# phazei/ComfyUI-HunyuanVideo-Foley

Hardware: AMD Instinct MI355X
Metric: audio-sec/sec (5s clip, 50-step Euler, CFG 4.5) (higher is better)
Workload: dtype bf16; 1 GPU; c2: T2A 5 s, 50 Euler steps, CFG 4.5, hunyuanvideo-foley-xxl, bs=1/GPU, bf16 GEMM operands / fp32 accumulate, weight storage none, DAC-VAE fp32 decode to 48 kHz, host-to-host (H2D noise + D2H waveform timed); clips_per_gpu=1, parallelism=dp1, hip_graph=True, progress_callback=False, collectives=0, bundle_bytes=10565004032, rccl_nranks=1

## Files before the change

comfyui-hunyuanvideo-foley_amd/csrc/attention.hip:

```cpp
#include <type_traits>

#include "kernels.h"

namespace {


template <int HD> __device__ constexpr float attn_scale() {
  return HD == 128 ? 0.08838834764831845f : HD == 64 ? 0.125f : 0.10206207261596575f;
}

__device__ __forceinline__ void attn_block_coords(const AttnArgs& a, int qtile, int& qt, int& h, int& b) {
  const int nq = (a.Sq + qtile - 1) / qtile;
  const int nwg = nq * a.H * a.Bq;
  int bid = (int)blockIdx.x;
  const int xcd = bid & 7, slot = bid >> 3;
  const int q = nwg >> 3, r = nwg & 7;
  bid = ((xcd < r) ? xcd * (q + 1) : r * (q + 1) + (xcd - r) * q) + slot;
  qt = bid % nq;
  const int bh = bid / nq;
  h = bh % a.H;
  b = bh / a.H;
}

template <typename OutT> struct Pack4Out;
template <> struct Pack4Out<float> {
  static __device__ __forceinline__ void store(float* p, const f32x4 v) { *(f32x4*)p = v; }
};
template <> struct Pack4Out<bf16_t> {
  static __device__ __forceinline__ void store(bf16_t* p, const f32x4 v) {
    uint2 w;
    w.x = pack_bf16x2(v[0], v[1]);
    w.y = pack_bf16x2(v[2], v[3]);
    *(uint2*)p = w;
  }
};

template <> struct Pack4Out<f16_t> {
  static __device__ __forceinline__ void store(f16_t* p, const f32x4 v) {
    uint2 w;
    w.x = pack_f16x2(v[0], v[1]);
    w.y = pack_f16x2(v[2], v[3]);
    *(uint2*)p = w;
  }
};

template <typename OutT, int HD>
__global__ __launch_bounds__(64) void attn_kernel(const AttnArgs a) {
  const int lane = threadIdx.x;
  const int j = lane & 31, kh = lane >> 5;
  const int q0 = blockIdx.x * 32;
  const int h = blockIdx.y, b = blockIdx.z;
  const int bk = b / a.kv_bdiv;
  const float* __restrict__ Q = (const float*)a.q + ((long)(b * a.H + h) * a.Sq) * HD;
  const float* __restrict__ K = (const float*)a.k + ((long)(bk * a.H + h) * a.Skv) * HD;
  const float* __restrict__ V = (const float*)a.v + ((long)(bk * a.H + h) * a.Skv) * HD;
  const float scale = attn_scale<HD>();

  constexpr int HH = HD / 2, NC = HD / 8;
  float qr[HH];
  {
    const int qrow = min(q0 + j, a.Sq - 1);
    const f32x4* p = (const f32x4*)(Q + (long)qrow * HD + kh * HH);
#pragma unroll
    for (int c = 0; c < NC; ++c) {
      const f32x4 v = p[c];
      qr[c * 4 + 0] = v[0]; qr[c * 4 + 1] = v[1]; qr[c * 4 + 2] = v[2]; qr[c * 4 + 3] = v[3];
    }
  }

  constexpr int ND = HD / 32;
  f32x16 o[ND];
#pragma unroll
  for (int d = 0; d < ND; ++d)
#pragma unroll
    for (int e = 0; e < 16; ++e) o[d][e] = 0.f;
  float m_run = -INFINITY, l_run = 0.f;

  for (int kt = 0; kt < a.Skv; kt += 32) {
    f32x16 s;
#pragma unroll
    for (int e = 0; e < 16; ++e) s[e] = 0.f;
    {
      const int krow = min(kt + j, a.Skv - 1);
      const f32x4* p = (const f32x4*)(K + (long)krow * HD + kh * HH);
#pragma unroll
      for (int c = 0; c < NC; ++c) {
        const f32x4 v = p[c];
        s = __builtin_amdgcn_mfma_f32_32x32x2f32(v[0], qr[c * 4 + 0], s, 0, 0, 0);
        s = __builtin_amdgcn_mfma_f32_32x32x2f32(v[1], qr[c * 4 + 1], s, 0, 0, 0);
        s = __builtin_amdgcn_mfma_f32_32x32x2f32(v[2], qr[c * 4 + 2], s, 0, 0, 0);
        s = __builtin_amdgcn_mfma_f32_32x32x2f32(v[3], qr[c * 4 + 3], s, 0, 0, 0);
      }
    }
    float mx = -INFINITY;
#pragma unroll
    for (int e = 0; e < 16; ++e) {
      const int key = kt + (e & 3) + 8 * (e >> 2) + 4 * kh;
      s[e] = (key < a.Skv) ? s[e] * scale : -INFINITY;
      mx = fmaxf(mx, s[e]);
    }
    mx = xhalf_max(mx);
    const float m_new = fmaxf(m_run, mx);
    const float alpha = expf(m_run - m_new);
    float ps = 0.f;
#pragma unroll
    for (int e = 0; e < 16; ++e) {
      s[e] = expf(s[e] - m_new);
      ps += s[e];
    }
    ps = xhalf_sum(ps);
    l_run = l_run * alpha + ps;
    m_run = m_new;
#pragma unroll
    for (int d = 0; d < ND; ++d)
#pragma unroll
      for (int e = 0; e < 16; ++e) o[d][e] *= alpha;
#pragma unroll
    for (int t = 0; t < 16; ++t) {
      const int vrow = min(kt + (t & 3) + 8 * (t >> 2) + 4 * kh, a.Skv - 1);
      const float* vp = V + (long)vrow * HD + j;
#pragma unroll
      for (int d = 0; d < ND; ++d)
        o[d] = __builtin_amdgcn_mfma_f32_32x32x2f32(vp[d * 32], s[t], o[d], 0, 0, 0);
    }
  }

  const int tok = q0 + j;
  if (tok >= a.Sq) return;
  const float inv = 1.0f / l_run;
  OutT* dst;
  if (HD == 64 && a.out_rows) {
    const int orow = a.out_rows[(long)b * a.Sq + tok];
    if ((unsigned)orow >= (unsigned)a.out_nrows) return;
    dst = (OutT*)a.outA + (long)orow * (a.H * HD);
  }
  else if (tok < a.split) dst = (OutT*)a.outA + ((long)b * a.split + tok) * (a.H * HD);
  else dst = (OutT*)a.outB + ((long)b * (a.Sq - a.split) + (tok - a.split)) * (a.H * HD);
  dst += h * HD;
#pragma unroll
  for (int d = 0; d < ND; ++d)
#pragma unroll
    for (int g4 = 0; g4 < 4; ++g4) {
      const int c = d * 32 + 8 * g4 + 4 * kh;
#pragma unroll
      for (int u = 0; u < 4; ++u) dst[c + u] = Cvt<OutT>::to(o[d][g4 * 4 + u] * inv);
    }
}

template <typename T, typename OutT>
__global__ __launch_bounds__(256) void attn_bf16_kernel(const AttnArgs a) {
  constexpr int HD = 128;
  __shared__ float sO[4][3][16][64];
  __shared__ float sM[4][32], sL[4][32];
  const int lane = threadIdx.x & 63, w = threadIdx.x >> 6;
  const int j = lane & 31, kh = lane >> 5;
  int qt, h, b;
  attn_block_coords(a, 32, qt, h, b);
  const int q0 = qt * 32;
  const int bk = b / a.kv_bdiv;
  const T* __restrict__ Q = (const T*)a.q + ((long)(b * a.H + h) * a.Sq) * HD;
  const T* __restrict__ K = (const T*)a.k + ((long)(bk * a.H + h) * a.Skv) * HD;
  const T* __restrict__ VT = (const T*)a.v + ((long)(bk * a.H + h) * HD) * a.vt_pitch;
  const float scale2 = 0.08838834764831845f * 1.4426950408889634f;

  const bool stamp = a.dbg && threadIdx.x == 0;
  if (stamp) a.dbg[(long)blockIdx.x * 8 + 0] = wall_clock64();
  bf16x8 qf[8];
  {
    const T* p = Q + (long)min(q0 + j, a.Sq - 1) * HD + 8 * kh;
#pragma unroll
    for (int s = 0; s < 8; ++s) qf[s] = *(const bf16x8*)(p + 16 * s);
  }
  f32x16 o[4];
#pragma unroll
  for (int d = 0; d < 4; ++d)
#pragma unroll
    for (int e = 0; e < 16; ++e) o[d][e] = 0.f;
  float m_run = -INFINITY, l_run = 0.f;

  const int nt = (a.Skv + 31) >> 5;
  const int t0 = (nt * w) >> 2, t1 = (nt * (w + 1)) >> 2;
  const int pi = 16 * ((j >> 2) & 1) + (j & 3) + 4 * (j >> 3);
  auto tile = [&](int kt, const bf16x8 (&kf)[8], const bf16x8 (&vf)[2][4]) {
    f32x16 s;
#pragma unroll
    for (int e = 0; e < 16; ++e) s[e] = 0.f;
#pragma unroll
    for (int st = 0; st < 8; ++st) s = mfma16<T>(kf[st], qf[st], s);
    float mx = -INFINITY;
#pragma unroll
    for (int e = 0; e < 16; ++e) {
      s[e] = (kt + 16 * kh + e < a.Skv) ? s[e] * scale2 : -INFINITY;
      mx = fmaxf(mx, s[e]);
    }
    mx = xhalf_max(mx);
    const float m_new = fmaxf(m_run, mx);
    float ps = 0.f;
    bf16x8 pb[2];
#pragma unroll
    for (int e = 0; e < 16; ++e) {
      const float pv = __builtin_amdgcn_exp2f(s[e] - m_new);
      ps += pv;
      pb[e >> 3][e & 7] = to_carrier<T>(pv);
    }
    ps = xhalf_sum(ps);
    if (__builtin_amdgcn_ballot_w64(m_new > m_run) != 0) {
      const float alpha = __builtin_amdgcn_exp2f(m_run - m_new);
      l_run *= alpha;
#pragma unroll
      for (int d = 0; d < 4; ++d)
#pragma unroll
        for (int e = 0; e < 16; ++e) o[d][e] *= alpha;
    }
    l_run += ps;
    m_run = m_new;
#pragma unroll
    for (int u = 0; u < 2; ++u)
#pragma unroll
      for (int d = 0; d < 4; ++d) o[d] = mfma16<T>(vf[u][d], pb[u], o[d]);
  };
  auto load_k = [&](int kt, bf16x8 (&kf)[8]) {
    const T* p = K + (long)min(kt + pi, a.Skv - 1) * HD + 8 * kh;
#pragma unroll
    for (int st = 0; st < 8; ++st) kf[st] = *(const bf16x8*)(p + 16 * st);
  };
  auto load_v = [&](int kt, bf16x8 (&vf)[2][4]) {
#pragma unroll
    for (int u = 0; u < 2; ++u)
#pragma unroll
      for (int d = 0; d < 4; ++d) vf[u][d] = *(const bf16x8*)(VT + (long)(d * 32 + j) * a.vt_pitch + kt + 16 * kh + 8 * u);
  };
  if (t1 - t0 <= 2) {
    bf16x8 k0[8], k1[8], v0[2][4], v1[2][4];
    const int kta = t0 * 32, ktb = min(t0 + 1, nt - 1) * 32;
    if (t1 > t0) {
      load_k(kta, k0);
      load_k(ktb, k1);
      load_v(kta, v0);
      load_v(ktb, v1);
      if (a.dbg) {
        asm volatile("s_waitcnt vmcnt(0)" ::: "memory");
        if (stamp) a.dbg[(long)blockIdx.x * 8 + 1] = wall_clock64();
      }
      tile(kta, k0, v0);
      if (t1 - t0 == 2) tile(ktb, k1, v1);
    }
  } else {
    for (int t = t0; t < t1; ++t) {
      bf16x8 kf[8], vf[2][4];
      load_k(t * 32, kf);
      load_v(t * 32, vf);
      tile(t * 32, kf, vf);
    }
  }

  if (stamp) a.dbg[(long)blockIdx.x * 8 + 2] = wall_clock64();
  if (kh == 0) {
    sM[w][j] = m_run;
    sL[w][j] = l_run;
  }
#pragma unroll
  for (int d = 0; d < 4; ++d) {
    if (d == w) continue;
    const int slot = d < w ? d : d - 1;
#pragma unroll
    for (int e = 0; e < 16; ++e) sO[w][slot][e][lane] = o[d][e];
  }
  __syncthreads();
  if (stamp) a.dbg[(long)blockIdx.x * 8 + 3] = wall_clock64();
  float mstar = -INFINITY;
#pragma unroll
  for (int x = 0; x < 4; ++x) mstar = fmaxf(mstar, sM[x][j]);
  float wt[4], L = 0.f;
#pragma unroll
  for (int x = 0; x < 4; ++x) {
    wt[x] = __builtin_amdgcn_exp2f(sM[x][j] - mstar);
    L += wt[x] * sL[x][j];
  }
  const int tok = q0 + j;
  if (tok >= a.Sq) return;
  const float inv = 1.0f / L;
  OutT* dst;
  if (tok < a.split) dst = (OutT*)a.outA + ((long)b * a.split + tok) * (a.H * HD);
  else dst = (OutT*)a.outB + ((long)b * (a.Sq - a.split) + (tok - a.split)) * (a.H * HD);
  dst += h * HD + w * 32;
  const int slot_mine = 0;
  (void)slot_mine;
  auto finish = [&](auto wc) {
    constexpr int W = decltype(wc)::value;
    float part[3][16];
#pragma unroll
    for (int x = 0, n = 0; x < 4; ++x) {
      if (x == W) continue;
      const int slot = W < x ? W : W - 1;
#pragma unroll
      for (int e = 0; e < 16; ++e) part[n][e] = sO[x][slot][e][lane];
      ++n;
    }
#pragma unroll
    for (int g4 = 0; g4 < 4; ++g4) {
      f32x4 r;
#pragma unroll
      for (int u = 0; u < 4; ++u) {
        const int e = g4 * 4 + u;
        float acc = 0.f;
#pragma unroll
        for (int x = 0, n = 0; x < 4; ++x) {
          if (x == W) acc += wt[x] * o[W][e];
          else acc += wt[x] * part[n++][e];
        }
        r[u] = acc * inv;
      }
      Pack4Out<OutT>::store(dst + 8 * g4 + 4 * kh, r);
    }
  };
  switch (__builtin_amdgcn_readfirstlane(w)) {
    case 0: finish(std::integral_constant<int, 0>{}); break;
    case 1: finish(std::integral_constant<int, 1>{}); break;
    case 2: finish(std::integral_constant<int, 2>{}); break;
    default: finish(std::integral_constant<int, 3>{}); break;
  }
  if (stamp) a.dbg[(long)blockIdx.x * 8 + 4] = wall_clock64();
}

__device__ __forceinline__ void attn_buf_lds16(const void* base, unsigned bytes, unsigned char* lds_wave_base, int voff) {
  const __amdgpu_buffer_rsrc_t r = __builtin_amdgcn_make_buffer_rsrc((void*)base, 0, (int)bytes, 0x00020000);
  __builtin_amdgcn_raw_ptr_buffer_load_lds(r, (__attribute__((address_space(3))) void*)lds_wave_base, 16, voff, 0, 0, 0);
}

template <typename T, typename OutT>
__global__ __launch_bounds__(256) void attn_lds_kernel(const AttnArgs a, const int merge_off) {
  constexpr int HD = 128;
  extern __shared__ __attribute__((aligned(16))) unsigned char dsm[];
  float (*sO)[3][16][64] = (float (*)[3][16][64])(dsm + merge_off);
  float (*sM)[32] = (float (*)[32])(dsm + merge_off + 4 * 3 * 16 * 64 * 4);
  float (*sL)[32] = (float (*)[32])(dsm + merge_off + 4 * 3 * 16 * 64 * 4 + 4 * 32 * 4);
  const int lane = threadIdx.x & 63, w = threadIdx.x >> 6;
  const int j = lane & 31, kh = lane >> 5;
  int qt, h, b;
  attn_block_coords(a, 32, qt, h, b);
  const int q0 = qt * 32;
  const int bk = b / a.kv_bdiv;
  const T* __restrict__ Q = (const T*)a.q + ((long)(b * a.H + h) * a.Sq) * HD;
  const T* __restrict__ K = (const T*)a.k + ((long)(bk * a.H + h) * a.Skv) * HD;
  const T* __restrict__ VT = (const T*)a.v + ((long)(bk * a.H + h) * HD) * a.vt_pitch;
  const float scale2 = 0.08838834764831845f * 1.4426950408889634f;

  const bool stamp = a.dbg && threadIdx.x == 0;
  if (stamp) a.dbg[(long)blockIdx.x * 8 + 0] = wall_clock64();
  const int nt = (a.Skv + 31) >> 5;
  const int lgCV = a.vt_pitch > 128 ? 5 : 4;
  unsigned char* const Ks = dsm;
  unsigned char* const Vs = Ks + nt * 32 * 256;
  unsigned char* const Qs = Vs + (128 << (lgCV + 4));
  const int wv = __builtin_amdgcn_readfirstlane(w);
  {
    const int r4 = lane >> 4, c16 = lane & 15;
    for (int p = wv; p < nt * 8; p += 4) {
      const int row = 4 * p + r4;
      const int g = c16 ^ ((row & 7) | ((row >> 1) & 8));
      attn_buf_lds16(K, (unsigned)a.Skv * 256u, Ks + p * 1024, row * 256 + g * 16);
    }
    const int vchunks = a.vt_pitch >> 3;
    for (int p = wv; p < (128 << lgCV) >> 6; p += 4) {
      const int pos = p * 64 + lane;
      const int row = pos >> lgCV, g = (pos & ((1 << lgCV) - 1)) ^ (row & 15);
      attn_buf_lds16(VT, (unsigned)(HD * a.vt_pitch * 2), Vs + p * 1024, g < vchunks ? (row * a.vt_pitch + g * 8) * 2 : 0x7ffffff0);
    }
    for (int p = wv; p < 8; p += 4) {
      const int row = 4 * p + r4;
      attn_buf_lds16(Q + (long)q0 * HD, (unsigned)(a.Sq - q0) * 256u, Qs + p * 1024, row * 256 + ((c16 ^ (row & 15)) << 4));
    }
  }
  asm volatile("s_waitcnt vmcnt(0)" ::: "memory");
  __syncthreads();
  if (stamp) a.dbg[(long)blockIdx.x * 8 + 1] = wall_clock64();
  bf16x8 qf[8];
#pragma unroll
  for (int s = 0; s < 8; ++s) qf[s] = *(const bf16x8*)(Qs + j * 256 + (((2 * s + kh) ^ (j & 15)) << 4));
  f32x16 o[4];
#pragma unroll
  for (int d = 0; d < 4; ++d)
#pragma unroll
    for (int e = 0; e < 16; ++e) o[d][e] = 0.f;
  float m_run = -INFINITY, l_run = 0.f;

  const int t0 = (nt * w) >> 2, t1 = (nt * (w + 1)) >> 2;
  const int pi = 16 * ((j >> 2) & 1) + (j & 3) + 4 * (j >> 3);
  auto tile = [&](int kt, const bf16x8 (&kf)[8], const bf16x8 (&vf)[2][4]) {
    f32x16 s;
#pragma unroll
    for (int e = 0; e < 16; ++e) s[e] = 0.f;
#pragma unroll
    for (int st = 0; st < 8; ++st) s = mfma16<T>(kf[st], qf[st], s);
    float mx = -INFINITY;
#pragma unroll
    for (int e = 0; e < 16; ++e) {
      s[e] = (kt + 16 * kh + e < a.Skv) ? s[e] * scale2 : -INFINITY;
      mx = fmaxf(mx, s[e]);
    }
    mx = xhalf_max(mx);
    const float m_new = fmaxf(m_run, mx);
    float ps = 0.f;
    bf16x8 pb[2];
#pragma unroll
    for (int e = 0; e < 16; ++e) {
      const float pv = __builtin_amdgcn_exp2f(s[e] - m_new);
      ps += pv;
      pb[e >> 3][e & 7] = to_carrier<T>(pv);
    }
    ps = xhalf_sum(ps);
    if (__builtin_amdgcn_ballot_w64(m_new > m_run) != 0) {
      const float alpha = __builtin_amdgcn_exp2f(m_run - m_new);
      l_run *= alpha;
#pragma unroll
      for (int d = 0; d < 4; ++d)
#pragma unroll
        for (int e = 0; e < 16; ++e) o[d][e] *= alpha;
    }
    l_run += ps;
    m_run = m_new;
#pragma unroll
    for (int u = 0; u < 2; ++u)
#pragma unroll
      for (int d = 0; d < 4; ++d) o[d] = mfma16<T>(vf[u][d], pb[u], o[d]);
  };
  const int pk = (pi & 7) | ((pi >> 1) & 8);
  auto read_k = [&](int kt, bf16x8 (&kf)[8]) {
    const unsigned char* kr = Ks + (kt + pi) * 256;
#pragma unroll
    for (int st = 0; st < 8; ++st) kf[st] = *(const bf16x8*)(kr + (((2 * st + kh) ^ pk) << 4));
  };
  auto read_v = [&](int kt, bf16x8 (&vf)[2][4]) {
#pragma unroll
    for (int u = 0; u < 2; ++u)
#pragma unroll
      for (int d = 0; d < 4; ++d) {
        const int row = d * 32 + j;
        vf[u][d] = *(const bf16x8*)(Vs + (row << (lgCV + 4)) + ((((kt >> 3) + 2 * kh + u) ^ (row & 15)) << 4));
      }
  };
  if (t1 - t0 <= 2) {
    bf16x8 k0[8], k1[8], v0[2][4], v1[2][4];
    const int kta = t0 * 32, ktb = min(t0 + 1, nt - 1) * 32;
    if (t1 > t0) {
      read_k(kta, k0);
      read_k(ktb, k1);
      read_v(kta, v0);
      read_v(ktb, v1);
      tile(kta, k0, v0);
      if (t1 - t0 == 2) tile(ktb, k1, v1);
    }
  } else {
    for (int t = t0; t < t1; ++t) {
      bf16x8 kf[8], vf[2][4];
      read_k(t * 32, kf);
      read_v(t * 32, vf);
      tile(t * 32, kf, vf);
    }
  }

  if (stamp) a.dbg[(long)blockIdx.x * 8 + 2] = wall_clock64();
  if (merge_off == 0) __syncthreads();
  if (kh == 0) {
    sM[w][j] = m_run;
    sL[w][j] = l_run;
  }
#pragma unroll
  for (int d = 0; d < 4; ++d) {
    if (d == w) continue;
    const int slot = d < w ? d : d - 1;
#pragma unroll
    for (int e = 0; e < 16; ++e) sO[w][slot][e][lane] = o[d][e];
  }
  __syncthreads();
  if (stamp) a.dbg[(long)blockIdx.x * 8 + 3] = wall_clock64();
  float mstar = -INFINITY;
#pragma unroll
  for (int x = 0; x < 4; ++x) mstar = fmaxf(mstar, sM[x][j]);
  float wt[4], L = 0.f;
#pragma unroll
  for (int x = 0; x < 4; ++x) {
    wt[x] = __builtin_amdgcn_exp2f(sM[x][j] - mstar);
    L += wt[x] * sL[x][j];
  }
  const int tok = q0 + j;
  if (tok >= a.Sq) return;
  const float inv = 1.0f / L;
  OutT* dst;
  if (tok < a.split) dst = (OutT*)a.outA + ((long)b * a.split + tok) * (a.H * HD);
  else dst = (OutT*)a.outB + ((long)b * (a.Sq - a.split) + (tok - a.split)) * (a.H * HD);
  dst += h * HD + w * 32;
  const int slot_mine = 0;
  (void)slot_mine;
  auto finish = [&](auto wc) {
    constexpr int W = decltype(wc)::value;
    float part[3][16];
#pragma unroll
    for (int x = 0, n = 0; x < 4; ++x) {
      if (x == W) continue;
      const int slot = W < x ? W : W - 1;
#pragma unroll
      for (int e = 0; e < 16; ++e) part[n][e] = sO[x][slot][e][lane];
      ++n;
    }
#pragma unroll
    for (int g4 = 0; g4 < 4; ++g4) {
      f32x4 r;
#pragma unroll
      for (int u = 0; u < 4; ++u) {
        const int e = g4 * 4 + u;
        float acc = 0.f;
#pragma unroll
        for (int x = 0, n = 0; x < 4; ++x) {
          if (x == W) acc += wt[x] * o[W][e];
          else acc += wt[x] * part[n++][e];
        }
        r[u] = acc * inv;
      }
      Pack4Out<OutT>::store(dst + 8 * g4 + 4 * kh, r);
    }
  };
  switch (__builtin_amdgcn_readfirstlane(w)) {
    case 0: finish(std::integral_constant<int, 0>{}); break;
    case 1: finish(std::integral_constant<int, 1>{}); break;
    case 2: finish(std::integral_constant<int, 2>{}); break;
    default: finish(std::integral_constant<int, 3>{}); break;
  }
  if (stamp) a.dbg[(long)blockIdx.x * 8 + 4] = wall_clock64();
}

template <typename T, typename OutT, int HD, bool GRP = false>
__global__ __launch_bounds__(256) __attribute__((amdgpu_waves_per_eu(3, 3))) void attn_bf16_wide_kernel(const AttnArgs a) {
  constexpr int KP = 2 * HD + 16, VP = 80;
  constexpr int STG = 32 * KP + HD * VP;
  constexpr int NS = HD / 16, ND = HD / 32;
  constexpr int CK = HD / 8, NP = HD / 64;
  __shared__ __attribute__((aligned(16))) unsigned char lds[2 * STG];
  const int tid = threadIdx.x, lane = tid & 63, w = tid >> 6;
  const int j = lane & 31, kh = lane >> 5;
  int qt, h, b;
  attn_block_coords(a, 128, qt, h, b);
  const int q0 = qt * 128 + w * 32;
  const int bk = b / a.kv_bdiv;
  const T* __restrict__ Q = (const T*)a.q + ((long)(b * a.H + h) * a.Sq) * HD;
  const T* __restrict__ K = (const T*)a.k + ((long)(bk * a.H + h) * a.Skv) * HD;
  const T* __restrict__ VT = (const T*)a.v + ((long)(bk * a.H + h) * HD) * a.vt_pitch;
  const float scale2 = attn_scale<HD>() * 1.4426950408889634f;

  bf16x8 qf[NS];
  {
    const T* p = Q + (long)min(q0 + j, a.Sq - 1) * HD + 8 * kh;
#pragma unroll
    for (int s = 0; s < NS; ++s) qf[s] = *(const bf16x8*)(p + 16 * s);
  }
  f32x16 o[ND];
#pragma unroll
  for (int d = 0; d < ND; ++d)
#pragma unroll
    for (int e = 0; e < 16; ++e) o[d][e] = 0.f;
  float m_run = -INFINITY, l_run = 0.f;
  int klo = 0, khi = 0, wlo = 0, whi = 0;
  if constexpr (GRP) {
    const int qi = min(q0 + j, a.Sq - 1);
    klo = (qi / a.grp_q) * a.grp_kv;
    khi = klo + a.grp_kv;
    if (q0 < a.Sq) {
      wlo = (q0 / a.grp_q) * a.grp_kv;
      whi = (min(q0 + 31, a.Sq - 1) / a.grp_q + 1) * a.grp_kv;
    }
  }

  const int k_row0 = tid / CK, k_col = tid % CK;
  const int v_row0 = tid >> 2, v_col = tid & 3;
  constexpr int NPX = HD % 64 ? 2 : NP;
  u32x4 rk[NPX], rv[NPX];
  auto gload = [&](int t) {
    const int kt = t * 32;
    if constexpr (HD % 64 == 0) {
#pragma unroll
      for (int i = 0; i < NP; ++i) {
        rk[i] = *(const u32x4*)(K + (long)min(kt + k_row0 + i * (256 / CK), a.Skv - 1) * HD + k_col * 8);
        rv[i] = *(const u32x4*)(VT + (long)(v_row0 + i * 64) * a.vt_pitch + kt + v_col * 8);
      }
    } else {
#pragma unroll
      for (int i = 0; i < NPX; ++i) {
        const int p = tid + 256 * i;
        if (p < 4 * HD) {
          rk[i] = *(const u32x4*)(K + (long)min(kt + p / CK, a.Skv - 1) * HD + (p % CK) * 8);
          rv[i] = *(const u32x4*)(VT + (long)(p >> 2) * a.vt_pitch + kt + (p & 3) * 8);
        }
      }
    }
  };
  auto lstore = [&](int stage) {
    unsigned char* base = lds + stage * STG;
    if constexpr (HD % 64 == 0) {
#pragma unroll
      for (int i = 0; i < NP; ++i) {
        *(u32x4*)(base + (k_row0 + i * (256 / CK)) * KP + k_col * 16) = rk[i];
        *(u32x4*)(base + 32 * KP + (v_row0 + i * 64) * VP + v_col * 16) = rv[i];
      }
    } else {
#pragma unroll
      for (int i = 0; i < NPX; ++i) {
        const int p = tid + 256 * i;
        if (p < 4 * HD) {
          *(u32x4*)(base + (p / CK) * KP + (p % CK) * 16) = rk[i];
          *(u32x4*)(base + 32 * KP + (p >> 2) * VP + (p & 3) * 16) = rv[i];
        }
      }
    }
  };
  const int nt = (a.Skv + 31) >> 5;
  const int pi = 16 * ((j >> 2) & 1) + (j & 3) + 4 * (j >> 3);
  const bool acct = a.dbg && tid == 0;
  long long c_math = 0, c_stage = 0, c_t0 = acct ? (long long)__builtin_readcyclecounter() : 0;
  gload(0);
  lstore(0);
  __syncthreads();
  for (int t = 0; t < nt; ++t) {
    const int kt = t * 32;
    const long long ca = acct ? (long long)__builtin_readcyclecounter() : 0;
    if (t + 1 < nt) gload(t + 1);
    const unsigned char* Ks = lds + (t & 1) * STG;
    const unsigned char* Vs = Ks + 32 * KP;
    bool live = true;
    if constexpr (GRP) live = kt < whi && kt + 32 > wlo;
    if (live) {
    f32x16 s;
#pragma unroll
    for (int e = 0; e < 16; ++e) s[e] = 0.f;
#pragma unroll
    for (int st = 0; st < NS; ++st)
      s = mfma16<T>(*(const bf16x8*)(Ks + pi * KP + (16 * st + 8 * kh) * 2), qf[st], s);
    float mx = -INFINITY;
    if constexpr (GRP) {
#pragma unroll
      for (int e = 0; e < 16; ++e) {
        const int key = kt + 16 * kh + e;
        s[e] = (key >= klo && key < khi) ? s[e] : -INFINITY;
      }
    } else if (kt + 32 > a.Skv) {
#pragma unroll
      for (int e = 0; e < 16; ++e) s[e] = (kt + 16 * kh + e < a.Skv) ? s[e] : -INFINITY;
    }
#pragma unroll
    for (int e = 0; e < 16; ++e) mx = fmaxf(mx, s[e]);
    mx = xhalf_max(mx);
    const float m_new = fmaxf(m_run, mx * scale2);
    const float m_exp = (GRP && m_new == -INFINITY) ? 0.f : m_new;
    float ps = 0.f;
    bf16x8 pb[2];
#pragma unroll
    for (int e = 0; e < 16; ++e) {
      const float pv = __builtin_amdgcn_exp2f(__builtin_fmaf(s[e], scale2, -m_exp));
      ps += pv;
      pb[e >> 3][e & 7] = to_carrier<T>(pv);
    }
    ps = xhalf_sum(ps);
    if (__builtin_amdgcn_ballot_w64(m_new > m_run) != 0) {
      const float alpha = (GRP && m_new == -INFINITY) ? 1.f : __builtin_amdgcn_exp2f(m_run - m_new);
      l_run *= alpha;
#pragma unroll
      for (int d = 0; d < ND; ++d)
#pragma unroll
        for (int e = 0; e < 16; ++e) o[d][e] *= alpha;
    }
    l_run += ps;
    m_run = m_new;
#pragma unroll
    for (int u = 0; u < 2; ++u)
#pragma unroll
      for (int d = 0; d < ND; ++d)
        o[d] = mfma16<T>(*(const bf16x8*)(Vs + (d * 32 + j) * VP + (16 * kh + 8 * u) * 2), pb[u], o[d]);
    }
    const long long cb = acct ? (long long)__builtin_readcyclecounter() : 0;
    if (t + 1 < nt) {
      lstore((t + 1) & 1);
      __syncthreads();
    }
    if (acct) {
      const long long cc = (long long)__builtin_readcyclecounter();
      c_math += cb - ca;
      c_stage += cc - cb;
    }
  }
  if (acct) {
    a.dbg[(long)blockIdx.x * 8 + 0] = (long long)__builtin_readcyclecounter() - c_t0;
    a.dbg[(long)blockIdx.x * 8 + 1] = c_math;
    a.dbg[(long)blockIdx.x * 8 + 2] = c_stage;
    a.dbg[(long)blockIdx.x * 8 + 3] = nt;
  }

  const int tok = q0 + j;
  if (tok >= a.Sq) return;
  const float inv = 1.0f / l_run;
  OutT* dst;
  if (HD == 64 && a.out_rows) {
    const int orow = a.out_rows[(long)b * a.Sq + tok];
    if ((unsigned)orow >= (unsigned)a.out_nrows) return;
    dst = (OutT*)a.outA + (long)orow * (a.H * HD);
  }
  else if (tok < a.split) dst = (OutT*)a.outA + ((long)b * a.split + tok) * (a.H * HD);
  else dst = (OutT*)a.outB + ((long)b * (a.Sq - a.split) + (tok - a.split)) * (a.H * HD);
  dst += h * HD;
#pragma unroll
  for (int d = 0; d < ND; ++d)
#pragma unroll
    for (int g4 = 0; g4 < 4; ++g4) {
      const f32x4 v = {o[d][g4 * 4 + 0] * inv, o[d][g4 * 4 + 1] * inv, o[d][g4 * 4 + 2] * inv, o[d][g4 * 4 + 3] * inv};
      Pack4Out<OutT>::store(dst + d * 32 + 8 * g4 + 4 * kh, v);
    }
}

template <typename T, typename OutT>
__global__ __launch_bounds__(256, 2) void attn_bf16_long_kernel(const AttnArgs a) {
  constexpr int HD = 128, KT = 64;
  constexpr int KP = 2 * HD + 16, VP = 2 * KT + 16;
  constexpr int STG = KT * KP + HD * VP;
  constexpr int NS = HD / 16, ND = HD / 32;
  extern __shared__ __attribute__((aligned(16))) unsigned char lds[];
  const int tid = threadIdx.x, lane = tid & 63, w = tid >> 6;
  const int j = lane & 31, kh = lane >> 5;
  int qt, h, b;
  attn_block_coords(a, 128, qt, h, b);
  const int q0 = qt * 128 + w * 32;
  const int bk = b / a.kv_bdiv;
  const T* __restrict__ Q = (const T*)a.q + ((long)(b * a.H + h) * a.Sq) * HD;
  const T* __restrict__ K = (const T*)a.k + ((long)(bk * a.H + h) * a.Skv) * HD;
  const T* __restrict__ VT = (const T*)a.v + ((long)(bk * a.H + h) * HD) * a.vt_pitch;
  const float scale2 = 0.08838834764831845f * 1.4426950408889634f;

  bf16x8 qf[NS];
  {
    const T* p = Q + (long)min(q0 + j, a.Sq - 1) * HD + 8 * kh;
#pragma unroll
    for (int s = 0; s < NS; ++s) qf[s] = *(const bf16x8*)(p + 16 * s);
  }
  f32x16 o[ND];
#pragma unroll
  for (int d = 0; d < ND; ++d)
#pragma unroll
    for (int e = 0; e < 16; ++e) o[d][e] = 0.f;
  float m_run = -INFINITY, l_run = 0.f;

  const int k_row0 = tid >> 4, k_col = tid & 15;
  const int v_row0 = tid >> 3, v_col = tid & 7;
  const int vmax = a.vt_pitch - 8;
  u32x4 rk[4], rv[4];
  auto gload = [&](int t) {
    const int kt = t * KT;
#pragma unroll
    for (int i = 0; i < 4; ++i) {
      rk[i] = *(const u32x4*)(K + (long)min(kt + k_row0 + i * 16, a.Skv - 1) * HD + k_col * 8);
      rv[i] = *(const u32x4*)(VT + (long)(v_row0 + i * 32) * a.vt_pitch + min(kt + v_col * 8, vmax));
    }
  };
  auto lstore = [&](int stage) {
    unsigned char* base = lds + stage * STG;
#pragma unroll
    for (int i = 0; i < 4; ++i) {
      *(u32x4*)(base + (k_row0 + i * 16) * KP + k_col * 16) = rk[i];
      *(u32x4*)(base + KT * KP + (v_row0 + i * 32) * VP + v_col * 16) = rv[i];
    }
  };
  const int nt = (a.Skv + KT - 1) / KT;
  const int pi = 16 * ((j >> 2) & 1) + (j & 3) + 4 * (j >> 3);
  gload(0);
  lstore(0);
  __syncthreads();
  for (int t = 0; t < nt; ++t) {
    const int kt = t * KT;
    if (t + 1 < nt) gload(t + 1);
    const unsigned char* Ks = lds + (t & 1) * STG;
    const unsigned char* Vs = Ks + KT * KP;
    f32x16 s0, s1;
#pragma unroll
    for (int e = 0; e < 16; ++e) s0[e] = s1[e] = 0.f;
#pragma unroll
    for (int st = 0; st < NS; ++st) {
      s0 = mfma16<T>(*(const bf16x8*)(Ks + pi * KP + (16 * st + 8 * kh) * 2), qf[st], s0);
      s1 = mfma16<T>(*(const bf16x8*)(Ks + (32 + pi) * KP + (16 * st + 8 * kh) * 2), qf[st], s1);
    }
    if (kt + KT > a.Skv) {
#pragma unroll
      for (int e = 0; e < 16; ++e) {
        s0[e] = (kt + 16 * kh + e < a.Skv) ? s0[e] : -INFINITY;
        s1[e] = (kt + 32 + 16 * kh + e < a.Skv) ? s1[e] : -INFINITY;
      }
    }
    float mx = -INFINITY;
#pragma unroll
    for (int e = 0; e < 16; ++e) mx = fmaxf(mx, fmaxf(s0[e], s1[e]));
    mx = xhalf_max(mx);
    const float m_new = fmaxf(m_run, mx * scale2);
    float ps = 0.f;
    bf16x8 pb[4];
#pragma unroll
    for (int e = 0; e < 16; ++e) {
      const float p0 = __builtin_amdgcn_exp2f(__builtin_fmaf(s0[e], scale2, -m_new));
      const float p1 = __builtin_amdgcn_exp2f(__builtin_fmaf(s1[e], scale2, -m_new));
      ps += p0 + p1;
      pb[e >> 3][e & 7] = to_carrier<T>(p0);
      pb[2 + (e >> 3)][e & 7] = to_carrier<T>(p1);
    }
    ps = xhalf_sum(ps);
    if (__builtin_amdgcn_ballot_w64(m_new > m_run) != 0) {
      const float alpha = __builtin_amdgcn_exp2f(m_run - m_new);
      l_run *= alpha;
#pragma unroll
      for (int d = 0; d < ND; ++d)
#pragma unroll
        for (int e = 0; e < 16; ++e) o[d][e] *= alpha;
    }
    l_run += ps;
    m_run = m_new;
#pragma unroll
    for (int u = 0; u < 4; ++u)
#pragma unroll
      for (int d = 0; d < ND; ++d)
        o[d] = mfma16<T>(*(const bf16x8*)(Vs + (d * 32 + j) * VP + (32 * (u >> 1) + 16 * kh + 8 * (u & 1)) * 2), pb[u], o[d]);
    if (t + 1 < nt) {
      lstore((t + 1) & 1);
      __syncthreads();
    }
  }

  const int tok = q0 + j;
  if (tok >= a.Sq) return;
  const float inv = 1.0f / l_run;
  OutT* dst;
  if (tok < a.split) dst = (OutT*)a.outA + ((long)b * a.split + tok) * (a.H * HD);
  else dst = (OutT*)a.outB + ((long)b * (a.Sq - a.split) + (tok - a.split)) * (a.H * HD);
  dst += h * HD;
#pragma unroll
  for (int d = 0; d < ND; ++d)
#pragma unroll
    for (int g4 = 0; g4 < 4; ++g4) {
      const f32x4 v = {o[d][g4 * 4 + 0] * inv, o[d][g4 * 4 + 1] * inv, o[d][g4 * 4 + 2] * inv, o[d][g4 * 4 + 3] * inv};
      Pack4Out<OutT>::store(dst + d * 32 + 8 * g4 + 4 * kh, v);
    }
}

template <typename T, typename OutT, int NQ>
__global__ __launch_bounds__(NQ * 128) void attn_bf16_pair_kernel(const AttnArgs a) {
  constexpr int HD = 128, KT = 64, NTH = NQ * 128;
  constexpr int KP = 2 * HD + 16, VP = 2 * KT + 16;
  constexpr int STG = KT * KP + HD * VP;
  constexpr int NS = HD / 16, ND = HD / 32;
  constexpr int NPC = (1024 + NTH - 1) / NTH;
  extern __shared__ __attribute__((aligned(16))) unsigned char lds[];
  const int tid = threadIdx.x, lane = tid & 63;
  const int w = __builtin_amdgcn_readfirstlane(tid >> 6);
  const int qb = w % NQ, kh2 = w / NQ;
  const int j = lane & 31, kh = lane >> 5;
  int qt, h, b;
  attn_block_coords(a, 32 * NQ, qt, h, b);
  const int q0 = qt * (32 * NQ) + qb * 32;
  const int bk = b / a.kv_bdiv;
  const T* __restrict__ Q = (const T*)a.q + ((long)(b * a.H + h) * a.Sq) * HD;
  const T* __restrict__ K = (const T*)a.k + ((long)(bk * a.H + h) * a.Skv) * HD;
  const T* __restrict__ VT = (const T*)a.v + ((long)(bk * a.H + h) * HD) * a.vt_pitch;
  const float scale2 = 0.08838834764831845f * 1.4426950408889634f;

  bf16x8 qf[NS];
  {
    const T* p = Q + (long)min(q0 + j, a.Sq - 1) * HD + 8 * kh;
#pragma unroll
    for (int s = 0; s < NS; ++s) qf[s] = *(const bf16x8*)(p + 16 * s);
  }
  f32x16 o[ND];
#pragma unroll
  for (int d = 0; d < ND; ++d)
#pragma unroll
    for (int e = 0; e < 16; ++e) o[d][e] = 0.f;
  float m_run = -INFINITY, l_run = 0.f;

  const int vmax = a.vt_pitch - 8;
  u32x4 rk[NPC], rv[NPC];
  auto gload = [&](int t) {
    const int kt = t * KT;
#pragma unroll
    for (int i = 0; i < NPC; ++i) {
      const int p = tid + i * NTH;
      if (p < 1024) {
        rk[i] = *(const u32x4*)(K + (long)min(kt + (p >> 4), a.Skv - 1) * HD + (p & 15) * 8);
        rv[i] = *(const u32x4*)(VT + (long)(p >> 3) * a.vt_pitch + min(kt + (p & 7) * 8, vmax));
      }
    }
  };
  auto lstore = [&](int stage) {
    unsigned char* base = lds + stage * STG;
#pragma unroll
    for (int i = 0; i < NPC; ++i) {
      const int p = tid + i * NTH;
      if (p < 1024) {
        *(u32x4*)(base + (p >> 4) * KP + (p & 15) * 16) = rk[i];
        *(u32x4*)(base + KT * KP + (p >> 3) * VP + (p & 7) * 16) = rv[i];
      }
    }
  };
  const int nt = (a.Skv + KT - 1) / KT;
  const int pi = 16 * ((j >> 2) & 1) + (j & 3) + 4 * (j >> 3);
  f32x16 s;
  auto qk = [&](int stg) {
    const unsigned char* Ks = lds + stg * STG + (32 * kh2) * KP;
#pragma unroll
    for (int e = 0; e < 16; ++e) s[e] = 0.f;
#pragma unroll
    for (int st = 0; st < NS; ++st) s = mfma16<T>(*(const bf16x8*)(Ks + pi * KP + (16 * st + 8 * kh) * 2), qf[st], s);
  };
  auto softmax_pv = [&](int t, int stg) {
    const int kt = t * KT + 32 * kh2;
    const unsigned char* Vs = lds + stg * STG + KT * KP + (32 * kh2) * 2;
    if (kt + 32 > a.Skv) {
#pragma unroll
      for (int e = 0; e < 16; ++e) s[e] = (kt + 16 * kh + e < a.Skv) ? s[e] : -INFINITY;
    }
    float mx = -INFINITY;
#pragma unroll
    for (int e = 0; e < 16; ++e) mx = fmaxf(mx, s[e]);
    mx = xhalf_max(mx);
    const float m_new = fmaxf(m_run, mx * scale2);
    float ps = 0.f;
    bf16x8 pb[2];
#pragma unroll
    for (int e = 0; e < 16; ++e) {
      const float pv = __builtin_amdgcn_exp2f(__builtin_fmaf(s[e], scale2, -m_new));
      ps += pv;
      pb[e >> 3][e & 7] = to_carrier<T>(pv);
    }
    ps = xhalf_sum(ps);
    if (__builtin_amdgcn_ballot_w64(m_new > m_run) != 0) {
      const float alpha = __builtin_amdgcn_exp2f(m_run - m_new);
      l_run *= alpha;
#pragma unroll
      for (int d = 0; d < ND; ++d)
#pragma unroll
        for (int e = 0; e < 16; ++e) o[d][e] *= alpha;
    }
    l_run += ps;
    m_run = m_new;
#pragma unroll
    for (int u = 0; u < 2; ++u)
#pragma unroll
      for (int d = 0; d < ND; ++d)
        o[d] = mfma16<T>(*(const bf16x8*)(Vs + (d * 32 + j) * VP + (16 * kh + 8 * u) * 2), pb[u], o[d]);
  };
  gload(0);
  lstore(0);
  __syncthreads();
  for (int t = 0; t < nt; ++t) {
    if (t + 1 < nt) gload(t + 1);
    if (t * KT + 32 * kh2 < a.Skv) {
      qk(t & 1);
      softmax_pv(t, t & 1);
    }
    if (t + 1 < nt) {
      lstore((t + 1) & 1);
      __syncthreads();
    }
  }
  __syncthreads();
  float* xm = (float*)lds + qb * (66 * 64);
  if (kh2 == 1) {
    xm[lane] = m_run;
    xm[64 + lane] = l_run;
#pragma unroll
    for (int d = 0; d < ND; ++d)
#pragma unroll
      for (int v = 0; v < 4; ++v) {
        const f32x4 t4 = {o[d][4 * v], o[d][4 * v + 1], o[d][4 * v + 2], o[d][4 * v + 3]};
        *(f32x4*)(xm + 128 + ((d * 4 + v) * 64 + lane) * 4) = t4;
      }
  }
  __syncthreads();
  if (kh2 == 1) return;
  {
    const float m_b = xm[lane], l_b = xm[64 + lane];
    const float m = fmaxf(m_run, m_b);
    const float fa = __builtin_amdgcn_exp2f(m_run - m), fb = __builtin_amdgcn_exp2f(m_b - m);
    l_run = l_run * fa + l_b * fb;
#pragma unroll
    for (int d = 0; d < ND; ++d)
#pragma unroll
      for (int v = 0; v < 4; ++v) {
        const f32x4 t4 = *(const f32x4*)(xm + 128 + ((d * 4 + v) * 64 + lane) * 4);
#pragma unroll
        for (int e = 0; e < 4; ++e) o[d][4 * v + e] = o[d][4 * v + e] * fa + t4[e] * fb;
      }
  }
  const int tok = q0 + j;
  if (tok >= a.Sq) return;
  const float inv = 1.0f / l_run;
  OutT* dst;
  if (tok < a.split) dst = (OutT*)a.outA + ((long)b * a.split + tok) * (a.H * HD);
  else dst = (OutT*)a.outB + ((long)b * (a.Sq - a.split) + (tok - a.split)) * (a.H * HD);
  dst += h * HD;
#pragma unroll
  for (int d = 0; d < ND; ++d)
#pragma unroll
    for (int g4 = 0; g4 < 4; ++g4) {
      const f32x4 v = {o[d][g4 * 4 + 0] * inv, o[d][g4 * 4 + 1] * inv, o[d][g4 * 4 + 2] * inv, o[d][g4 * 4 + 3] * inv};
      Pack4Out<OutT>::store(dst + d * 32 + 8 * g4 + 4 * kh, v);
    }
}

}

static long long* g_attn_dbg = nullptr;
extern "C" void foley_debug_attn_timeline(void* p) { g_attn_dbg = (long long*)p; }

int launch_attention(const AttnArgs& a_in, int out_dtype, hipStream_t st) {
  AttnArgs a = a_in;
  a.dbg = g_attn_dbg;
  if (a.Sq <= 0 || a.Skv <= 0) return foley_set_err("attention: empty sequence", __FILE__, __LINE__);
  const int hd = a.head_dim > 0 ? a.head_dim : 128;
  if (hd != 128 && hd != 64 && hd != 96) return foley_set_err("attention: head_dim must be 128, 96 or 64", __FILE__, __LINE__);
  if (a.grp_q > 0 || a.grp_kv > 0) {
    if (hd != 64 || !foley_is_half(a.in_dtype) || a.grp_q < 1 || a.grp_kv < 1 || a.kv_bdiv != 1 ||
        (long)((a.Sq + a.grp_q - 1) / a.grp_q) * a.grp_kv > a.Skv)
      return foley_set_err("attention: grouped (block-diagonal) form: head_dim 64, 16-bit operands, every query group's keys inside Skv", __FILE__, __LINE__);
  }
  if (a.out_rows && hd != 64) return foley_set_err("attention: the output row table serves head_dim 64 (the conditioning encoders' kernels)", __FILE__, __LINE__);
  dim3 grid((a.Sq + 31) / 32, a.H, a.Bq), block(64);
  const dim3 grid1(grid.x * grid.y * grid.z);
  if (foley_is_half(a.in_dtype)) {
    if (a.vt_pitch < ((a.Skv + 31) & ~31) || (a.vt_pitch & 7))
      return foley_set_err("attention: V^T pitch must cover Skv rounded up to 32 (multiple of 8)", __FILE__, __LINE__);
    if (out_dtype != a.in_dtype && out_dtype != FOLEY_F32)
      return foley_set_err("attention: 16-bit operands produce the same type or fp32", __FILE__, __LINE__);
    const dim3 gw(((a.Sq + 127) / 128) * a.H * a.Bq);
    const bool wide = (long)gw.x >= 256 || hd != 128, h16 = a.in_dtype == FOLEY_F16, o32 = out_dtype == FOLEY_F32;
    const bool longk = wide && hd == 128 && a.Skv >= 512 && (long)gw.x * 4 <= 2048;
    int pair_nq = 0;
    if (longk) {
      long best = 0;
      for (int nq = 6; nq >= 4; --nq) {
        const long wgs = (long)((a.Sq + 32 * nq - 1) / (32 * nq)) * a.H * a.Bq;
        if (wgs <= 256 && wgs > best) { best = wgs; pair_nq = nq; }
      }
      if (best < 160) pair_nq = 0;
    }
    const int nt = (a.Skv + 31) >> 5;
    const long img = (long)nt * 32 * 256 + (128L << ((a.vt_pitch > 128 ? 5 : 4) + 4)) + 32 * 256, mrg = 4 * 3 * 16 * 64 * 4 + 2 * 4 * 32 * 4;
    const bool staged = !wide && hd == 128 && nt >= 4 && a.vt_pitch <= 256 && img <= 160 * 1024;
    const int merge_off = staged && img + mrg <= 160 * 1024 ? (int)img : 0;
    const size_t lds16 = staged ? (size_t)(merge_off ? img + mrg : (img > mrg ? img : mrg)) : 0;
#define FOLEY_ATTN16(T, O)                                                                         \
    do {                                                                                             \
      if (staged) {                                                                                  \
        static std::atomic<unsigned long long> raised{0};                                            \
        hipError_t e_ = foley_raise_lds((const void*)attn_lds_kernel<T, O>, 160 * 1024, raised);     \
        if (e_ != hipSuccess) return foley_set_err(hipGetErrorString(e_), __FILE__, __LINE__);       \
        FOLEY_LAUNCH((attn_lds_kernel<T, O>), grid1, dim3(256), lds16, st, a, merge_off);            \
      } else                                                                                         \
      if (pair_nq) {                                                                                 \
        static std::atomic<unsigned long long> r4{0}, r5{0}, r6{0};                                  \
        const dim3 gp(((a.Sq + 32 * pair_nq - 1) / (32 * pair_nq)) * a.H * a.Bq);                    \
        hipError_t e_ = hipSuccess;                                                                  \
        if (pair_nq == 6) { e_ = foley_raise_lds((const void*)attn_bf16_pair_kernel<T, O, 6>, 6 * 16896, r6); if (e_ == hipSuccess) FOLEY_LAUNCH((attn_bf16_pair_kernel<T, O, 6>), gp, dim3(768), 6 * 16896, st, a); } \
        else if (pair_nq == 5) { e_ = foley_raise_lds((const void*)attn_bf16_pair_kernel<T, O, 5>, 5 * 16896, r5); if (e_ == hipSuccess) FOLEY_LAUNCH((attn_bf16_pair_kernel<T, O, 5>), gp, dim3(640), 5 * 16896, st, a); } \
        else { e_ = foley_raise_lds((const void*)attn_bf16_pair_kernel<T, O, 4>, 2 * 35840, r4); if (e_ == hipSuccess) FOLEY_LAUNCH((attn_bf16_pair_kernel<T, O, 4>), gp, dim3(512), 2 * 35840, st, a); } \
        if (e_ != hipSuccess) return foley_set_err(hipGetErrorString(e_), __FILE__, __LINE__);       \
      } else                                                                                         \
      if (longk) {                                                                                   \
        static std::atomic<unsigned long long> raised{0};                                            \
        hipError_t e_ = foley_raise_lds((const void*)attn_bf16_long_kernel<T, O>, 2 * 35840, raised); \
        if (e_ != hipSuccess) return foley_set_err(hipGetErrorString(e_), __FILE__, __LINE__);       \
        FOLEY_LAUNCH((attn_bf16_long_kernel<T, O>), gw, dim3(256), 2 * 35840, st, a);                \
      } else                                                                                         \
      if (wide && hd == 64 && a.grp_q > 0) FOLEY_LAUNCH((attn_bf16_wide_kernel<T, O, 64, true>), gw, dim3(256), 0, st, a);  \
      else if (wide && hd == 64) FOLEY_LAUNCH((attn_bf16_wide_kernel<T, O, 64>), gw, dim3(256), 0, st, a);  \
      else if (wide && hd == 96) FOLEY_LAUNCH((attn_bf16_wide_kernel<T, O, 96>), gw, dim3(256), 0, st, a);  \
      else if (wide) FOLEY_LAUNCH((attn_bf16_wide_kernel<T, O, 128>), gw, dim3(256), 0, st, a);        \
      else FOLEY_LAUNCH((attn_bf16_kernel<T, O>), grid1, dim3(256), 0, st, a);                         \
    } while (0)
    if (h16) { if (o32) FOLEY_ATTN16(f16_t, float); else FOLEY_ATTN16(f16_t, f16_t); }
    else { if (o32) FOLEY_ATTN16(bf16_t, float); else FOLEY_ATTN16(bf16_t, bf16_t); }
#undef FOLEY_ATTN16
    hipError_t e2 = hipGetLastError();
    if (e2 != hipSuccess) return foley_set_err(hipGetErrorString(e2), __FILE__, __LINE__);
    return 0;
  }
#define FOLEY_ATTN32(O)                                                          \
  do {                                                                           \
    if (hd == 64) FOLEY_LAUNCH((attn_kernel<O, 64>), grid, block, 0, st, a);     \
    else if (hd == 96) FOLEY_LAUNCH((attn_kernel<O, 96>), grid, block, 0, st, a); \
    else FOLEY_LAUNCH((attn_kernel<O, 128>), grid, block, 0, st, a);             \
  } while (0)
  if (out_dtype == FOLEY_F32) FOLEY_ATTN32(float);
  else if (out_dtype == FOLEY_BF16) FOLEY_ATTN32(bf16_t);
  else if (out_dtype == FOLEY_F16) FOLEY_ATTN32(f16_t);
  else return foley_set_err("attention: bad output dtype", __FILE__, __LINE__);
#undef FOLEY_ATTN32
  hipError_t e = hipGetLastError();
  if (e != hipSuccess) return foley_set_err(hipGetErrorString(e), __FILE__, __LINE__);
  return 0;
}
```

Before: 14.74 audio-sec/sec.

## Stream pair-attention K/V tiles directly to LDS with triple-buffered async pipeline

Replaces the register-staged global-to-LDS copy in the paired-wave attention kernel with direct buffer-to-LDS loads (attn_buf_lds16) into a three-stage ring. Tiles are issued two iterations ahead, and handover uses vmcnt waits plus a raw barrier. The padded LDS rows are replaced with XOR-swizzled layouts to avoid bank conflicts, and LDS addresses are precomputed per lane. The goal is to hide global latency and remove the register round trip and per-tile store pass. The cost is more LDS (at least 96 KB) and fragile hand-written waitcnt accounting.

After: 14.73 audio-sec/sec. No clear change (-0.1%).

```diff
diff --git a/comfyui-hunyuanvideo-foley_amd/csrc/attention.hip b/comfyui-hunyuanvideo-foley_amd/csrc/attention.hip
--- a/comfyui-hunyuanvideo-foley_amd/csrc/attention.hip
+++ b/comfyui-hunyuanvideo-foley_amd/csrc/attention.hip
@@ -846,11 +846,11 @@
 
 template <typename T, typename OutT, int NQ>
 __global__ __launch_bounds__(NQ * 128) void attn_bf16_pair_kernel(const AttnArgs a) {
-  constexpr int HD = 128, KT = 64, NTH = NQ * 128;
-  constexpr int KP = 2 * HD + 16, VP = 2 * KT + 16;
-  constexpr int STG = KT * KP + HD * VP;
+  constexpr int HD = 128, KT = 64, NW = 2 * NQ;
+  constexpr int TB = KT * HD * 2;
+  constexpr int NSTG = 3, VB = NSTG * TB;
   constexpr int NS = HD / 16, ND = HD / 32;
-  constexpr int NPC = (1024 + NTH - 1) / NTH;
+  constexpr int NPC = (32 + NW - 1) / NW;
   extern __shared__ __attribute__((aligned(16))) unsigned char lds[];
   const int tid = threadIdx.x, lane = tid & 63;
   const int w = __builtin_amdgcn_readfirstlane(tid >> 6);
@@ -879,42 +879,52 @@
   float m_run = -INFINITY, l_run = 0.f;
 
   const int vmax = a.vt_pitch - 8;
-  u32x4 rk[NPC], rv[NPC];
-  auto gload = [&](int t) {
+  const unsigned kbytes = (unsigned)a.Skv * (2 * HD), vbytes = (unsigned)(HD * a.vt_pitch * 2);
+  const int mine = (32 - w + NW - 1) / NW;
+  auto issue = [&](int t, int stg) {
     const int kt = t * KT;
 #pragma unroll
     for (int i = 0; i < NPC; ++i) {
-      const int p = tid + i * NTH;
-      if (p < 1024) {
-        rk[i] = *(const u32x4*)(K + (long)min(kt + (p >> 4), a.Skv - 1) * HD + (p & 15) * 8);
-        rv[i] = *(const u32x4*)(VT + (long)(p >> 3) * a.vt_pitch + min(kt + (p & 7) * 8, vmax));
-      }
-    }
-  };
-  auto lstore = [&](int stage) {
-    unsigned char* base = lds + stage * STG;
-#pragma unroll
-    for (int i = 0; i < NPC; ++i) {
-      const int p = tid + i * NTH;
-      if (p < 1024) {
-        *(u32x4*)(base + (p >> 4) * KP + (p & 15) * 16) = rk[i];
-        *(u32x4*)(base + KT * KP + (p >> 3) * VP + (p & 7) * 16) = rv[i];
-      }
-    }
+      const int p = w + i * NW;
+      if (p < 16) {
+        const int row = 4 * p + (lane >> 4);
+        const int g = (lane & 15) ^ ((row & 7) | ((row >> 1) & 8));
+        attn_buf_lds16(K, kbytes, lds + stg * TB + p * 1024, min(kt + row, a.Skv - 1) * (2 * HD) + g * 16);
+      } else if (p < 32) {
+        const int row = 8 * (p - 16) + (lane >> 3);
+        const int g = (lane & 7) ^ ((row >> 1) & 7);
+        attn_buf_lds16(VT, vbytes, lds + VB + stg * TB + (p - 16) * 1024, (row * a.vt_pitch + min(kt + g * 8, vmax)) * 2);
+      }
+    }
+  };
+  auto hand_over = [&](bool more) {
+    if (!more) asm volatile("s_waitcnt vmcnt(0) lgkmcnt(0)" ::: "memory");
+    else if (mine == NPC) asm volatile("s_waitcnt vmcnt(%0) lgkmcnt(0)" ::"n"(NPC) : "memory");
+    else asm volatile("s_waitcnt vmcnt(%0) lgkmcnt(0)" ::"n"(NPC - 1) : "memory");
+    __builtin_amdgcn_sched_barrier(0);
+    __builtin_amdgcn_s_barrier();
+    __builtin_amdgcn_sched_barrier(0);
+    asm volatile("" ::: "memory");
   };
   const int nt = (a.Skv + KT - 1) / KT;
   const int pi = 16 * ((j >> 2) & 1) + (j & 3) + 4 * (j >> 3);
+  const int pk = (pi & 7) | ((pi >> 1) & 8);
+  const unsigned char *ka[NS], *va[2];
+#pragma unroll
+  for (int st = 0; st < NS; ++st) ka[st] = lds + (32 * kh2 + pi) * (2 * HD) + (((2 * st + kh) ^ pk) << 4);
+#pragma unroll
+  for (int u = 0; u < 2; ++u) va[u] = lds + VB + j * (2 * KT) + (((4 * kh2 + 2 * kh + u) ^ ((j >> 1) & 7)) << 4);
   f32x16 s;
-  auto qk = [&](int stg) {
-    const unsigned char* Ks = lds + stg * STG + (32 * kh2) * KP;
+  auto qk = [&](auto sc) {
+    constexpr int S = decltype(sc)::value;
 #pragma unroll
     for (int e = 0; e < 16; ++e) s[e] = 0.f;
 #pragma unroll
-    for (int st = 0; st < NS; ++st) s = mfma16<T>(*(const bf16x8*)(Ks + pi * KP + (16 * st + 8 * kh) * 2), qf[st], s);
-  };
-  auto softmax_pv = [&](int t, int stg) {
+    for (int st = 0; st < NS; ++st) s = mfma16<T>(*(const bf16x8*)(ka[st] + S * TB), qf[st], s);
+  };
+  auto softmax_pv = [&](int t, auto sc) {
+    constexpr int S = decltype(sc)::value;
     const int kt = t * KT + 32 * kh2;
-    const unsigned char* Vs = lds + stg * STG + KT * KP + (32 * kh2) * 2;
     if (kt + 32 > a.Skv) {
 #pragma unroll
       for (int e = 0; e < 16; ++e) s[e] = (kt + 16 * kh + e < a.Skv) ? s[e] : -INFINITY;
@@ -947,21 +957,24 @@
     for (int u = 0; u < 2; ++u)
 #pragma unroll
       for (int d = 0; d < ND; ++d)
-        o[d] = mfma16<T>(*(const bf16x8*)(Vs + (d * 32 + j) * VP + (16 * kh + 8 * u) * 2), pb[u], o[d]);
-  };
-  gload(0);
-  lstore(0);
-  __syncthreads();
-  for (int t = 0; t < nt; ++t) {
-    if (t + 1 < nt) gload(t + 1);
+        o[d] = mfma16<T>(*(const bf16x8*)(va[u] + S * TB + d * (32 * 2 * KT)), pb[u], o[d]);
+  };
+  auto step = [&](auto sc, int t) {
+    constexpr int S = decltype(sc)::value;
+    if (t + 2 < nt) issue(t + 2, (S + 2) % NSTG);
     if (t * KT + 32 * kh2 < a.Skv) {
-      qk(t & 1);
-      softmax_pv(t, t & 1);
-    }
-    if (t + 1 < nt) {
-      lstore((t + 1) & 1);
-      __syncthreads();
-    }
+      qk(sc);
+      softmax_pv(t, sc);
+    }
+    if (t + 1 < nt) hand_over(t + 2 < nt);
+  };
+  issue(0, 0);
+  if (nt > 1) issue(1, 1);
+  hand_over(nt > 1);
+  for (int t = 0; t < nt; t += NSTG) {
+    step(std::integral_constant<int, 0>{}, t);
+    if (t + 1 < nt) step(std::integral_constant<int, 1>{}, t + 1);
+    if (t + 2 < nt) step(std::integral_constant<int, 2>{}, t + 2);
   }
   __syncthreads();
   float* xm = (float*)lds + qb * (66 * 64);
@@ -1044,6 +1057,7 @@
       }
       if (best < 160) pair_nq = 0;
     }
+    const int pair_lds = pair_nq * 16896 > 3 * 32768 ? pair_nq * 16896 : 3 * 32768;
     const int nt = (a.Skv + 31) >> 5;
     const long img = (long)nt * 32 * 256 + (128L << ((a.vt_pitch > 128 ? 5 : 4) + 4)) + 32 * 256, mrg = 4 * 3 * 16 * 64 * 4 + 2 * 4 * 32 * 4;
     const bool staged = !wide && hd == 128 && nt >= 4 && a.vt_pitch <= 256 && img <= 160 * 1024;
@@ -1061,9 +1075,9 @@
         static std::atomic<unsigned long long> r4{0}, r5{0}, r6{0};                                  \
         const dim3 gp(((a.Sq + 32 * pair_nq - 1) / (32 * pair_nq)) * a.H * a.Bq);                    \
         hipError_t e_ = hipSuccess;                                                                  \
-        if (pair_nq == 6) { e_ = foley_raise_lds((const void*)attn_bf16_pair_kernel<T, O, 6>, 6 * 16896, r6); if (e_ == hipSuccess) FOLEY_LAUNCH((attn_bf16_pair_kernel<T, O, 6>), gp, dim3(768), 6 * 16896, st, a); } \
-        else if (pair_nq == 5) { e_ = foley_raise_lds((const void*)attn_bf16_pair_kernel<T, O, 5>, 5 * 16896, r5); if (e_ == hipSuccess) FOLEY_LAUNCH((attn_bf16_pair_kernel<T, O, 5>), gp, dim3(640), 5 * 16896, st, a); } \
-        else { e_ = foley_raise_lds((const void*)attn_bf16_pair_kernel<T, O, 4>, 2 * 35840, r4); if (e_ == hipSuccess) FOLEY_LAUNCH((attn_bf16_pair_kernel<T, O, 4>), gp, dim3(512), 2 * 35840, st, a); } \
+        if (pair_nq == 6) { e_ = foley_raise_lds((const void*)attn_bf16_pair_kernel<T, O, 6>, pair_lds, r6); if (e_ == hipSuccess) FOLEY_LAUNCH((attn_bf16_pair_kernel<T, O, 6>), gp, dim3(768), pair_lds, st, a); } \
+        else if (pair_nq == 5) { e_ = foley_raise_lds((const void*)attn_bf16_pair_kernel<T, O, 5>, pair_lds, r5); if (e_ == hipSuccess) FOLEY_LAUNCH((attn_bf16_pair_kernel<T, O, 5>), gp, dim3(640), pair_lds, st, a); } \
+        else { e_ = foley_raise_lds((const void*)attn_bf16_pair_kernel<T, O, 4>, pair_lds, r4); if (e_ == hipSuccess) FOLEY_LAUNCH((attn_bf16_pair_kernel<T, O, 4>), gp, dim3(512), pair_lds, st, a); } \
         if (e_ != hipSuccess) return foley_set_err(hipGetErrorString(e_), __FILE__, __LINE__);       \
       } else                                                                                         \
       if (longk) {                                                                                   \
```
